# fishmarch/MS-SLAM

Hardware: AMD Instinct MI355X
Metric: Mkeypoints/s extract+describe, KITTI-00-like stereo 1241x376, 2000 feat/frame (higher is better)
Workload: dtype u8

## Files before the change

### ms-slam_amd/csrc/orb_kernels.hip

```cpp
#include <hip/hip_runtime.h>

#include <algorithm>
#include <string>
#include <stdint.h>
#include <stdlib.h>

#include "lds_limit.h"
#include "orb_device.h"
#include "gauss7_stream_device.h"
#include "sincosf_restated.h"

namespace msorb {

__global__ __launch_bounds__(256) void pyr_resize_kernel(LevelView src, LevelView dst, uint8_t* __restrict__ dst_base,
                                                         const ResizeTap* __restrict__ tx,
                                                         const ResizeTap* __restrict__ ty, int single_stage) {
    const int img = blockIdx.z;
    const int dy = blockIdx.y * 4 + (threadIdx.x >> 6);
    const int dx0 = (blockIdx.x * 64 + (threadIdx.x & 63)) * 4;
    if (dy >= dst.h || dx0 >= dst.w) return;
    const ResizeTap vy = ty[dy];
    const uint8_t* s0 = src.base + (size_t)img * src.img_stride + (size_t)vy.i0 * src.pitch;
    const uint8_t* s1 = src.base + (size_t)img * src.img_stride + (size_t)vy.i1 * src.pitch;
    const int b0 = vy.c0, b1 = vy.c1;
// ... 185 lines not shown
    static constexpr int kTileRows = 58;
    static constexpr int kTilePitch = 52;
    static constexpr int kScorePitch = 52;
    static constexpr int kScoreRows = 54;
    static constexpr int kMaxDet = 51;
    static constexpr int kWorkCap = 1536;
    static constexpr int kThreads = 128;
    static constexpr int kWordsPerRow = 2;
    static constexpr int kMaxR = 5;
    static constexpr int kMinWaves = 8;
};

__device__ __forceinline__ int min3i(int a, int b, int c) { return min(a, min(b, c)); }
__device__ __forceinline__ int max3i(int a, int b, int c) { return max(a, max(b, c)); }

#define MSORB_PK2(NAME, OPC)                                                                                                   \
    __device__ __forceinline__ uint32_t NAME(uint32_t a, uint32_t b) {                                                         \
        uint32_t r; asm(OPC " %0, %1, %2" : "=v"(r) : "v"(a), "v"(b)); return r; }                                             \
    __device__ __forceinline__ uint32_t NAME##_sw(uint32_t a, uint32_t b) {                            \
        uint32_t r; asm(OPC " %0, %1, %2 op_sel:[0,1] op_sel_hi:[1,0]" : "=v"(r) : "v"(a), "v"(b)); return r; }
MSORB_PK2(pk_min16, "v_pk_min_i16")
MSORB_PK2(pk_max16, "v_pk_max_i16")
#undef MSORB_PK2
__device__ __forceinline__ uint32_t pk_mad16(uint32_t a, uint32_t b, uint32_t c) {
    uint32_t r; asm("v_pk_mad_i16 %0, %1, %2, %3" : "=v"(r) : "v"(a), "v"(b), "v"(c)); return r;
}

template <class GEO>
__device__ __forceinline__ int fast_arc_contrast_pk(const uint8_t* p, int sgn) {
    constexpr int P = GEO::kTilePitch;
    const uint32_t sv = ((uint32_t)(sgn * (int)p[0]) & 0xffffu) * 0x10001u, ns = ((uint32_t)(-sgn) & 0xffffu) * 0x10001u;
    uint32_t D[8];
    D[0] = pk_mad16(((uint32_t)p[-3 * P] << 16) | p[3 * P], ns, sv);
    D[1] = pk_mad16(((uint32_t)p[-3 * P - 1] << 16) | p[3 * P + 1], ns, sv);
    D[2] = pk_mad16(((uint32_t)p[-2 * P - 2] << 16) | p[2 * P + 2], ns, sv);
    D[3] = pk_mad16(((uint32_t)p[-1 * P - 3] << 16) | p[1 * P + 3], ns, sv);
    D[4] = pk_mad16(((uint32_t)p[-3] << 16) | p[3], ns, sv);
    D[5] = pk_mad16(((uint32_t)p[1 * P - 3] << 16) | p[-1 * P + 3], ns, sv);
    D[6] = pk_mad16(((uint32_t)p[2 * P - 2] << 16) | p[-2 * P + 2], ns, sv);
    D[7] = pk_mad16(((uint32_t)p[3 * P - 1] << 16) | p[-3 * P + 1], ns, sv);
    const uint32_t m2_1 = pk_min16(D[1], D[2]), m2_3 = pk_min16(D[3], D[4]), m2_5 = pk_min16(D[5], D[6]),
                   m2_7 = pk_min16_sw(D[7], D[0]);
    const uint32_t m4_1 = pk_min16(m2_1, m2_3), m4_3 = pk_min16(m2_3, m2_5), m4_5 = pk_min16(m2_5, m2_7),
                   m4_7 = pk_min16_sw(m2_7, m2_1);
    const uint32_t c8_0 = pk_min16(m4_1, m4_5), c8_2 = pk_min16(m4_3, m4_7), c8_4 = pk_min16_sw(m4_5, m4_1),
                   c8_6 = pk_min16_sw(m4_7, m4_3);
    const uint32_t e0 = pk_max16_sw(D[0], D[1]), e2 = pk_max16_sw(D[2], D[3]), e4 = pk_max16_sw(D[4], D[5]),
                   e6 = pk_max16_sw(D[6], D[7]);
    const uint32_t a = pk_max16(pk_max16(pk_min16(c8_0, e0), pk_min16(c8_2, e2)), pk_max16(pk_min16(c8_4, e4), pk_min16(c8_6, e6)));
    return (int)(short)(pk_max16_sw(a, a) & 0xffffu);
}

__device__ __forceinline__ int wave_incl_scan(int v, int) {
    v += __builtin_amdgcn_update_dpp(0, v, 0x111 , 0xf, 0xf, false);
    v += __builtin_amdgcn_update_dpp(0, v, 0x112 , 0xf, 0xf, false);
    v += __builtin_amdgcn_update_dpp(0, v, 0x114 , 0xf, 0xf, false);
    v += __builtin_amdgcn_update_dpp(0, v, 0x118 , 0xf, 0xf, false);
    v += __builtin_amdgcn_update_dpp(0, v, 0x142 , 0xa, 0xf, false);
    v += __builtin_amdgcn_update_dpp(0, v, 0x143 , 0xc, 0xf, false);
    return v;
}

typedef short short2v __attribute__((ext_vector_type(2)));
__device__ __forceinline__ short2v as_s2(uint32_t v) { return __builtin_bit_cast(short2v, v); }
__device__ __forceinline__ uint32_t as_u32(short2v v) { return __builtin_bit_cast(uint32_t, v); }


template <int WAVES>
__device__ __forceinline__ int block_excl_scan(int cnt, int lane, int wave, int* wave_tot , int* total) {
    const int incl = wave_incl_scan(cnt, lane);
    if (lane == 63) wave_tot[wave] = incl;
    __syncthreads();
    int before = 0, tot = 0;
#pragma unroll
    for (int w = 0; w < WAVES; w++) {
        const int c = wave_tot[w];
        if (w < wave) before += c;
        tot += c;
    }
    *total = tot;
    return before + incl - cnt;
}

template <bool ALIGNED, class GEO>
__device__ __forceinline__ void fast_cells_body(const PyramidView& pyr, const CellDesc* __restrict__ cells, const FastThreadRec* __restrict__ ttab,
                                                         int ini_th, int min_th, int slots_per_image,
                                                         Cand16* __restrict__ slots, int* __restrict__ cell_count,
                                                         int n_cells, uint32_t gx_magic, const unsigned lin, const unsigned grid_x, const unsigned total) {
    constexpr int T = GEO::kThreads, P = GEO::kTilePitch, SP = GEO::kScorePitch;
    constexpr int kScoreBytes = (GEO::kScoreRows * SP + 15) & ~15;
    constexpr int kBitWords = GEO::kWordsPerRow * GEO::kMaxDet;
    static_assert(kBitWords <= T, "one bitmap word per thread");
    constexpr FastShape kShape = T == kFastSmall.threads ? kFastSmall : kFastLarge;
    static_assert(kShape.threads == T && kShape.tile_pitch == P && kShape.col_lanes == (P <= 64 ? 16 : 32), "orb_host.h FastShape");
    __shared__ __attribute__((aligned(16))) uint8_t tile_mem[kTileFront + GEO::kTileRows * P + 8];
    __shared__ __attribute__((aligned(16))) uint8_t score[kScoreBytes];
    __shared__ uint16_t work[GEO::kWorkCap];
    __shared__ int wave_tot[2][T / 64];
    __shared__ uint32_t kbits[kBitWords];
    __shared__ int kprefix[kBitWords];
    __shared__ uint16_t lut[32];
    __shared__ uint16_t tbase[T];
    uint8_t* const tile = tile_mem + kTileFront;

    const unsigned chunk = (total + 7) >> 3;
    unsigned wg = (lin & 7u) * chunk + (lin >> 3);
    if (total & 7u) wg = lin;
    const int img = gx_magic ? (int)__umulhi(wg, gx_magic) : (int)(wg / grid_x);
    const int cell_id = (int)(wg - (unsigned)img * grid_x);
    const CellDesc cd = cells[cell_id];
    const LevelView lv = pyr.lv[cd.level];
    const int rw = cd.rw, rh = cd.rh;
    const int dh = rh - 6;
    const int tid = threadIdx.x, lane = tid & 63, wave = tid >> 6;
    const int ga = cd.x0 & ~3;
    const int x_lo = cd.x0 + 3, x_hi = cd.x0 + rw - 3;
    const int gx0 = x_lo & ~3;
    const int G = cd.G;
    const int c_lo = gx0 - ga;
    const uint32_t magic = cd.g_magic;

    const uint8_t* src = lv.base + (size_t)img * lv.img_stride + (size_t)cd.y0 * lv.pitch;
    FastThreadRec tr{};
    if (ALIGNED) tr = ttab[cd.tt_off + (uint32_t)tid];
    if (ALIGNED) {
        constexpr int kColLanes = P <= 64 ? 16 : 32;
        constexpr int kRowsPerPass = T / kColLanes;
        constexpr int kPasses = (GEO::kTileRows - 1 + kRowsPerPass - 1) / kRowsPerPass;
        const int c = tid & (kColLanes - 1), r0 = tid / kColLanes;
        if (c < cd.ndw) {
            const uint32_t col = (uint32_t)(ga + 4 * c);
            const uint32_t pitch = (uint32_t)lv.pitch;
            const uint32_t off0 = __umul24((uint32_t)r0, pitch) + col, off_last = (uint32_t)(rh - 1) * pitch + col;
            uint32_t v[kPasses];
#pragma unroll
            for (int p = 0; p < kPasses; p++)
                v[p] = *reinterpret_cast<const uint32_t*>(src + min(off0 + (uint32_t)(p * kRowsPerPass) * pitch, off_last));
            uint8_t* l0 = &tile[tr.lds_store];
#pragma unroll
            for (int p = 0; p < kPasses; p++)
                if ((p + 1) * kRowsPerPass <= GEO::kTileRows || r0 + p * kRowsPerPass < GEO::kTileRows)
                    *reinterpret_cast<uint32_t*>(l0 + p * kRowsPerPass * P) = v[p];
        }
    } else {
        const int off = cd.x0 - ga;
        const uint32_t bmagic = cd.rw_magic;
        for (int i = tid; i < rh * rw; i += T) {
            const int y = (int)(__umul24((uint32_t)i, bmagic) >> 20), x = i - (int)__umul24((uint32_t)y, (uint32_t)rw);
            tile[(int)__umul24((uint32_t)y, P) + off + x] = src[(size_t)(__umul24((uint32_t)y, (uint32_t)lv.pitch) + (uint32_t)(cd.x0 + x))];
        }
    }
    auto clear_planes = [&]() {
#pragma unroll
        for (int k = 0; k < (kScoreBytes / 16 + T - 1) / T; k++)
            if ((k + 1) * T <= kScoreBytes / 16 || tid + k * T < kScoreBytes / 16)
                reinterpret_cast<uint4*>(score)[tid + k * T] = uint4{0, 0, 0, 0};
        if (tid < kBitWords) kbits[tid] = 0;
    };
    clear_planes();
    if (tid < 32) lut[tid] = (uint16_t)((((tid >> 1) & 3) << 7) + (tid >> 3) + ((tid & 1) << 15));

    const bool by_wave = (T == 128 ? cd.by_wave[0] : cd.by_wave[1]) != 0;
    const int sw = __builtin_amdgcn_readfirstlane(wave) * 8;
    const int R = !by_wave ? (T == 128 ? cd.R128 : cd.R256) : (int)(((T == 128 ? cd.rw128 : cd.rw256) >> sw) & 255u);
    int nrows;
    uint32_t Hm;
    uint32_t colp_off;
    uint32_t baseA;
    if (ALIGNED) {
        nrows = (int)(tr.rows_tbase & 0xffffu);
        Hm = tr.hm;
        colp_off = tr.colp;
        baseA = tr.rows_tbase >> 16;
    } else {
        int g_own, y_b;
        if (!by_wave) {
            const int strip = (int)(__umul24((uint32_t)tid, magic) >> 20);
            g_own = tid - strip * G;
            y_b = strip * R;
        } else {
            const int sl = (int)(__umul24((uint32_t)lane, magic) >> 20);
            g_own = lane - sl * G;
            const int y_w = (int)(((T == 128 ? cd.yw128 : cd.yw256) >> sw) & 255u);
            y_b = sl < (int)cd.spw ? y_w + sl * R : dh;
        }
        nrows = min(max(dh - y_b, 0), R);
        const int c_own = c_lo + 4 * g_own;
        const int xg = ga + c_own;
        const int vlo = min(max(x_lo - xg, 0), 4), vhi = min(max(x_hi - xg, 0), 4);
        Hm = (0x80808080u << (8 * vlo)) & (uint32_t)(0x0080808080ull >> (8 * (4 - vhi)));
        if (vlo >= 4) Hm = 0;
        colp_off = __umul24((uint32_t)y_b, P) + (uint32_t)c_own;
        baseA = (uint32_t)(((y_b + 3) << 7) | c_own);
    }
    tbase[tid] = (uint16_t)baseA;
    auto quick_test = [&](int th, uint32_t& wA, uint32_t& wB) {
        wA = 0; wB = 0;
        const uint8_t* colp = &tile[colp_off];
        uint32_t cw[GEO::kMaxR + 6], lw[GEO::kMaxR], rw_[GEO::kMaxR];
#pragma unroll
        for (int r = 0; r < GEO::kMaxR + 6; r++)
            if (r < 9 || r - 6 < R) cw[r] = *reinterpret_cast<const uint32_t*>(colp + r * P);
#pragma unroll
        for (int k = 0; k < GEO::kMaxR; k++)
            if (k < 3 || k < R) {
                lw[k] = *reinterpret_cast<const uint32_t*>(colp + (k + 3) * P - 4);
                rw_[k] = *reinterpret_cast<const uint32_t*>(colp + (k + 3) * P + 4);
            }
        const ushort2v t2 = __builtin_bit_cast(ushort2v, (uint32_t)th * 0x00010001u);
#pragma unroll
        for (int k = 0; k < GEO::kMaxR; k++) {
            if (k >= 3 && k >= R) break;
            const uint32_t V = cw[k + 3], U = cw[k], D = cw[k + 6];
            const uint32_t R3 = __builtin_amdgcn_alignbyte(rw_[k], V, 3);
            const uint32_t L3 = __builtin_amdgcn_alignbyte(V, lw[k], 1);
            const uint32_t Ve = V & 0x00ff00ffu, Vo = (V >> 8) & 0x00ff00ffu;
            const uint32_t Ae = __builtin_bit_cast(uint32_t, __builtin_elementwise_sub_sat(__builtin_bit_cast(ushort2v, Ve), t2));
            const uint32_t Ao = __builtin_bit_cast(uint32_t, __builtin_elementwise_sub_sat(__builtin_bit_cast(ushort2v, Vo), t2));
            const uint32_t Qd = ~(Ae | (Ao << 8));
            const uint32_t Be = __builtin_bit_cast(uint32_t, __builtin_elementwise_sub_sat(__builtin_bit_cast(ushort2v, Ve ^ 0x00ff00ffu), t2));
            const uint32_t Bo = __builtin_bit_cast(uint32_t, __builtin_elementwise_sub_sat(__builtin_bit_cast(ushort2v, Vo ^ 0x00ff00ffu), t2));
            const uint32_t Qb = Be | (Bo << 8);
            const uint32_t one = 0x01010101u;
            const uint32_t X = (__builtin_amdgcn_lerp(U, Qd, one) & __builtin_amdgcn_lerp(D, Qd, one)) |
                               (__builtin_amdgcn_lerp(L3, Qd, one) & __builtin_amdgcn_lerp(R3, Qd, one));
            const uint32_t Y = (__builtin_amdgcn_lerp(U, Qb, 0u) | __builtin_amdgcn_lerp(D, Qb, 0u)) &
                               (__builtin_amdgcn_lerp(L3, Qb, 0u) | __builtin_amdgcn_lerp(R3, Qb, 0u));
            const uint32_t hm = k < nrows ? Hm : 0u;
            const uint32_t z = (Y & hm) | ((~X & hm) >> 1);
            if (k < 4) wA |= z >> (6 - 2 * k);
            else wB |= z >> (6 - 2 * (k - 4));
        }
    };
    __syncthreads();

    const int sc_off = 4 - c_lo;
    Cand16* const out = slots + (size_t)img * slots_per_image + cd.slot_off;
    int n_emitted = 0;
    for (int pass = 0; pass < 2; pass++) {
        const int th = pass ? min_th : ini_th;
        uint32_t wA, wB;
        quick_test(th, wA, wB);
        const int cnt = __popc(wA) + __popc(wB);
        int n_work = 0;
        const int my_base = block_excl_scan<T / 64>(cnt, lane, wave, wave_tot[0], &n_work);

        const uint32_t baseB = baseA + (4u << 7);
        int w_begin = 0, n_corner = 0;
        if (n_work <= GEO::kWorkCap) {
            uint16_t* wp = &work[my_base];
            const uint32_t idA = (uint32_t)tid << 5, idB = idA | (1u << (5 + (T == 128 ? 7 : 8)));
            for (uint32_t w = wA; w; w &= w - 1) *wp++ = (uint16_t)(idA | (uint32_t)__builtin_ctz(w));
            for (uint32_t w = wB; w; w &= w - 1) *wp++ = (uint16_t)(idB | (uint32_t)__builtin_ctz(w));
            __syncthreads();
            w_begin = wave * ((((n_work + T / 64 - 1) / (T / 64)) + 63) & ~63);
            const int w_end = min(w_begin + ((((n_work + T / 64 - 1) / (T / 64)) + 63) & ~63), n_work);
            n_corner = 0;
            for (int i0 = w_begin; i0 < w_end; i0 += 64) {
                const int i = i0 + lane;
                bool corner = false;
                int ce = 0;
                if (i < w_end) {
                    const int id = work[i];
                    const int e = tbase[(id >> 5) & (T - 1)] + lut[id & 31] + ((id >> (5 + (T == 128 ? 7 : 8))) << 9);
                    const int ty = (e >> 7) & 127, tx = e & 127;
                    const int A = fast_arc_contrast_pk<GEO>(&tile[(int)__umul24((uint32_t)ty, P) + tx], (e & 0x8000) ? -1 : 1);
                    if (A > th) {
                        score[(int)__umul24((uint32_t)(ty - 2), SP) + tx + sc_off] = (uint8_t)(A - 1);
                        ce = e & 0x3FFF;
                        corner = true;
                    }
                }
                const unsigned long long bm = __ballot(corner);
                if (corner)
                    work[w_begin + n_corner + (int)__builtin_amdgcn_mbcnt_hi((uint32_t)(bm >> 32), __builtin_amdgcn_mbcnt_lo((uint32_t)bm, 0u))] = (uint16_t)ce;
                n_corner += __popcll(bm);
            }
        } else {
#pragma unroll 1
            for (int half = 0; half < 2; half++)
#pragma unroll 1
                for (uint32_t w = half ? wB : wA; w; w &= w - 1) {
                    const int e = lut[__builtin_ctz(w)] + (half ? baseB : baseA);
                    const int ty = (e >> 7) & 127, tx = e & 127;
                    const int A = fast_arc_contrast_pk<GEO>(&tile[(int)__umul24((uint32_t)ty, P) + tx], (e & 0x8000) ? -1 : 1);
                    if (A > th) score[(int)__umul24((uint32_t)(ty - 2), SP) + tx + sc_off] = (uint8_t)(A - 1);
                }
        }
        __syncthreads();

        if (n_work <= GEO::kWorkCap) {
            constexpr int wpr = GEO::kWordsPerRow;
            const int nwords = dh * wpr;
            uint32_t mine_keep = 0;
            {
                int slot = 0;
                for (int m0 = 0; m0 < n_corner; m0 += 64, slot++) {
                    if (m0 + lane >= n_corner) continue;
                    const int e = work[w_begin + m0 + lane];
                    const int ty = e >> 7, tx = e & 127;
                    const uint8_t* q = &score[(int)__umul24((uint32_t)(ty - 2), SP) + tx + sc_off];
                    const int sv = q[0];
                    int m = max3i(q[-SP - 1], q[-SP], q[-SP + 1]);
                    m = max3i(m, q[-1], q[1]);
                    m = max(m, max3i(q[SP - 1], q[SP], q[SP + 1]));
                    if (sv > m) {
                        const int bx = tx - c_lo, by = ty - 3;
                        const int b = by * (32 * wpr) + bx;
                        atomicOr(&kbits[b >> 5], 1u << (b & 31));
                        mine_keep |= 1u << slot;
                    }
                }
            }
            __syncthreads();
            const uint32_t myword = tid < nwords ? kbits[tid] : 0u;
            int n_out = 0;
            const int wprefix = block_excl_scan<T / 64>(__popc(myword), lane, wave, wave_tot[1], &n_out);
            if (tid < nwords) kprefix[tid] = wprefix;
            __syncthreads();
            {
                int slot = 0;
                for (int m0 = 0; m0 < n_corner; m0 += 64, slot++) {
                    if (!(mine_keep & (1u << slot))) continue;
                    const int e = work[w_begin + m0 + lane];
                    const int ty = e >> 7, tx = e & 127;
                    const int b = (ty - 3) * (32 * wpr) + (tx - c_lo);
                    const int rank = kprefix[b >> 5] + __popc(kbits[b >> 5] & ((1u << (b & 31)) - 1u));
                    Cand16 c;
                    c.x = (uint16_t)(ga + tx - kMinBorder);
                    c.y = (uint16_t)(cd.y0 + ty - kMinBorder);
                    c.score = score[(int)__umul24((uint32_t)(ty - 2), SP) + tx + sc_off];
                    c.pad = 0;
                    out[rank] = c;
                }
            }
            n_emitted = n_out;
        } else {
            const int n_task = dh * G;
            uint32_t tid_here = (uint32_t)tid;
            asm volatile("" : "+v"(tid_here));
            const int t_begin = (int)(__umul24(tid_here, (uint32_t)n_task) / T),
                      t_end = (int)(__umul24(tid_here + 1u, (uint32_t)n_task) / T);
            uint64_t keep = 0;
            {
                int y = (int)(__umul24((uint32_t)t_begin, magic) >> 20);
                int g = t_begin - y * G;
                for (int task = t_begin, k = 0; task < t_end; task++, k++) {
                    const uint8_t* sp = &score[(y + 1) * SP + 4 + 4 * g];
                    const uint32_t S = *reinterpret_cast<const uint32_t*>(sp);
                    if (S) {
#pragma unroll
                        for (int j = 0; j < 4; j++) {
                            const int sv = (S >> (8 * j)) & 255;
                            if (sv) {
                                const uint8_t* q = sp + j;
                                int m = max3i(q[-SP - 1], q[-SP], q[-SP + 1]);
                                m = max3i(m, q[-1], q[1]);
                                m = max(m, max3i(q[SP - 1], q[SP], q[SP + 1]));
                                if (sv > m) keep |= 1ull << (4 * k + j);
                            }
                        }
                    }
                    if (++g == G) { g = 0; y++; }
                }
            }
            int n_out = 0;
            int pos = block_excl_scan<T / 64>(__popcll(keep), lane, wave, wave_tot[1], &n_out);
            if (keep) {
                int y = (int)(__umul24((uint32_t)t_begin, magic) >> 20);
                int g = t_begin - y * G;
                uint64_t m = keep;
                for (int task = t_begin; task < t_end; task++, m >>= 4) {
                    uint32_t m4 = (uint32_t)m & 15u;
                    while (m4) {
                        const int j = __ffs(m4) - 1;
                        m4 &= m4 - 1;
                        Cand16 c;
                        c.x = (uint16_t)(gx0 + 4 * g + j - kMinBorder);
                        c.y = (uint16_t)(cd.y0 + 3 + y - kMinBorder);
                        c.score = score[(y + 1) * SP + 4 + 4 * g + j];
                        c.pad = 0;
                        out[pos++] = c;
                    }
                    if (++g == G) { g = 0; y++; }
                }
            }
            n_emitted = n_out;
        }
        if (n_emitted > 0 || pass == 1 || ini_th == min_th) break;
        __syncthreads();
        clear_planes();
        __syncthreads();
    }
    if (tid == 0) cell_count[(size_t)img * n_cells + cell_id] = n_emitted;
}

template <bool ALIGNED, class GEO>
__global__ __launch_bounds__(GEO::kThreads, GEO::kMinWaves) void fast_cells_kernel(PyramidView pyr, const CellDesc* __restrict__ cells,
                                                         const FastThreadRec* __restrict__ ttab,
                                                         int ini_th, int min_th, int slots_per_image,
                                                         Cand16* __restrict__ slots, int* __restrict__ cell_count,
                                                         int n_cells, uint32_t gx_magic) {
    fast_cells_body<ALIGNED, GEO>(pyr, cells, ttab, ini_th, min_th, slots_per_image, slots, cell_count, n_cells, gx_magic,
                                  blockIdx.y * gridDim.x + blockIdx.x, gridDim.x, gridDim.x * gridDim.y);
}

__global__ __launch_bounds__(256) void cand_scan_cells_kernel(const int* __restrict__ cell_count, int n_cells,
                                                              const int* __restrict__ level_cell_begin, int nlevels,
                                                              int* __restrict__ cell_off, int* __restrict__ level_count,
                                                              int* __restrict__ img_total, int* __restrict__ img_base,
                                                              int fixed_stride) {
    __shared__ int wave_tot[4];
    __shared__ int lvl[kMaxLevels];
    const int img = blockIdx.x, tid = threadIdx.x, lane = tid & 63, wave = tid >> 6;
    if (fixed_stride > 0 && tid == 0) {
        img_base[img] = img * fixed_stride;
        if (img == (int)gridDim.x - 1) img_base[gridDim.x] = (int)gridDim.x * fixed_stride;
    }
    const int* cnt = cell_count + (size_t)img * n_cells;
    int* off = cell_off + (size_t)img * n_cells;
    const int per = (n_cells + 255) / 256;
    const int b = tid * per, e = min(b + per, n_cells);
    constexpr int kCache = 4;
    int c[kCache];
#pragma unroll
    for (int k = 0; k < kCache; k++) c[k] = b + k < e ? cnt[b + k] : 0;
    int s = 0;
#pragma unroll
    for (int k = 0; k < kCache; k++) s += c[k];
    for (int i = b + kCache; i < e; i++) s += cnt[i];
    if (tid < kMaxLevels) lvl[tid] = 0;
    int total = 0;
    int acc = block_excl_scan<4>(s, lane, wave, wave_tot, &total);
    if (tid == 0) img_total[img] = total;
    int cur_l = 0, cur_t = 0;
    auto visit = [&](int i, int v) {
        off[i] = acc;
        acc += v;
        while (i >= level_cell_begin[cur_l + 1]) {
            if (cur_t) atomicAdd(&lvl[cur_l], cur_t);
            cur_t = 0;
            cur_l++;
        }
        cur_t += v;
    };
#pragma unroll
    for (int k = 0; k < kCache; k++)
        if (b + k < e) visit(b + k, c[k]);
    for (int i = b + kCache; i < e; i++) visit(i, cnt[i]);
    if (cur_t) atomicAdd(&lvl[cur_l], cur_t);
    __syncthreads();
    if (tid < nlevels) level_count[(size_t)img * nlevels + tid] = lvl[tid];
}

__global__ __launch_bounds__(256) void cand_scan_images_kernel(const int* __restrict__ img_total, int n_images,
                                                               int* __restrict__ img_base ) {
    __shared__ int wave_tot[4];
    const int tid = threadIdx.x, lane = tid & 63, wave = tid >> 6;
    const int per = (n_images + 255) / 256;
    const int b = tid * per, e = min(b + per, n_images);
    const int first = b < e ? img_total[b] : 0;
    int s = first;
    for (int i = b + 1; i < e; i++) s += img_total[i];
    int total = 0;
    int acc = block_excl_scan<4>(s, lane, wave, wave_tot, &total);
    if (tid == 0) img_base[n_images] = total;
    if (b < e) { img_base[b] = acc; acc += first; }
    for (int i = b + 1; i < e; i++) { img_base[i] = acc; acc += img_total[i]; }
}

constexpr int kGatherThreads = 256;
constexpr int kGatherCells = kGatherThreads / 16;
__global__ __launch_bounds__(kGatherThreads) void cand_gather_kernel(const CellDesc* __restrict__ cells, int n_cells,
                                                          int slots_per_image, const Cand16* __restrict__ slots,
                                                          const int* __restrict__ cell_count,
                                                          const int* __restrict__ cell_off,
                                                          const int* __restrict__ img_base, Cand16* __restrict__ compact) {
    const int c0 = blockIdx.x * kGatherCells + 2 * (int)(threadIdx.x >> 5), img = blockIdx.y, l = threadIdx.x & 31;
    if (c0 >= n_cells) return;
    const int c1 = min(c0 + 1, n_cells - 1);
    const int* cnt = cell_count + (size_t)img * n_cells;
    const int* off = cell_off + (size_t)img * n_cells;
    const int n0 = cnt[c0], n1 = c0 + 1 < n_cells ? cnt[c1] : 0;
    const int o0 = off[c0], o1 = off[c1], s0 = cells[c0].slot_off, s1 = cells[c1].slot_off, base = img_base[img];
    const Cand16* sp = slots + (size_t)img * slots_per_image;
    Cand16* d = compact + base;
    Cand16 v0{}, v1{};
// ... 88 lines not shown
    if (ALIGNED) {
        const uint32_t* ap = reinterpret_cast<const uint32_t*>(rp + x0);
        w1 = ap[0]; w2 = ap[1];
        w0 = x0 ? ap[-1] : 0u;
    } else {
        const uint32_t ph = (uint32_t)(reinterpret_cast<uintptr_t>(rp) & 3);
        const uint32_t* ap = reinterpret_cast<const uint32_t*>(rp - ph + x0);
        const uint32_t d1 = ap[0], d2 = ap[1], d3 = ap[2];
        const uint32_t d0 = x0 ? ap[-1] : 0u;
        w0 = __builtin_amdgcn_alignbyte(d1, d0, ph);
        w1 = __builtin_amdgcn_alignbyte(d2, d1, ph);
        w2 = __builtin_amdgcn_alignbyte(d3, d2, ph);
    }
    if (x0 == 0) w0 = __builtin_amdgcn_perm(0u, w1, 0x01020300u);
#pragma unroll
    for (int j = 0; j < 4; j++) {
        const uint32_t a = j == 3 ? w1 : __builtin_amdgcn_alignbyte(w1, w0, j + 1);
        const uint32_t b = j == 3 ? w2 : __builtin_amdgcn_alignbyte(w2, w1, j + 1);
        hsum[j] = __builtin_amdgcn_udot4(b, kGaussHi, __builtin_amdgcn_udot4(a, kGaussLo, 0u, false), false);
    }
}

template <bool ALIGNED>
__global__ __launch_bounds__(256) void gauss7_kernel(PyramidView src, PyramidView dst, BlurPlan plan, GaussTaps T) {
    const uint32_t K[7] = {T.k[0], T.k[1], T.k[2], T.k[3], T.k[4], T.k[5], T.k[6]};
    const uint32_t kGaussLo = K[0] | (K[1] << 8) | (K[2] << 16) | (K[3] << 24), kGaussHi = K[4] | (K[5] << 8) | (K[6] << 16);
    int level = 0;
    while (level + 1 < plan.nlevels && (int)blockIdx.x >= plan.block_begin[level + 1]) level++;
    const int rem = blockIdx.x - plan.block_begin[level];
    const int bx = rem % plan.bx_count[level], by = rem / plan.bx_count[level];
    const LevelView sv = src.lv[level], dv = dst.lv[level];
    const int img = blockIdx.y;
    const int x0 = (bx * 64 + (threadIdx.x & 63)) * 4;
    const int y0 = (by * 4 + (threadIdx.x >> 6)) * kGaussRows;
    if (x0 + 16 > sv.w || y0 >= sv.h) return;
    const uint8_t* sb = sv.base + (size_t)img * sv.img_stride;
    uint8_t* db = const_cast<uint8_t*>(dv.base) + (size_t)img * dv.img_stride;
    uint32_t acc[7][4];
    uint32_t hs[4];
#pragma unroll
    for (int r = 0; r < 6; r++) {
        gauss_row_sums<ALIGNED>(sb, sv.pitch, sv.h, y0 - 3 + r, x0, hs, kGaussLo, kGaussHi);
#pragma unroll
        for (int t = 0; t <= r; t++)
#pragma unroll
            for (int j = 0; j < 4; j++) acc[r - t][j] = (t == 0 ? 0u : acc[r - t][j]) + K[t] * hs[j];
    }
    for (int it = 0; it < kGaussRows / 7; it++) {
#pragma unroll
        for (int u = 0; u < 7; u++) {
            const int r = 6 + 7 * it + u;
            gauss_row_sums<ALIGNED>(sb, sv.pitch, sv.h, y0 - 3 + r, x0, hs, kGaussLo, kGaussHi);
#pragma unroll
            for (int t = 0; t < 7; t++) {
                const int a = (6 + u - t) % 7;
#pragma unroll
                for (int j = 0; j < 4; j++) acc[a][j] = (t == 0 ? 0u : acc[a][j]) + K[t] * hs[j];
            }
            const int o = r - 6, a = u % 7;
            if (y0 + o < sv.h) {
                uint32_t packed = 0;
#pragma unroll
                for (int j = 0; j < 4; j++) packed |= min((acc[a][j] + 32768u) >> 16, 255u) << (8 * j);
                *reinterpret_cast<uint32_t*>(db + blur_tile_off((uint32_t)x0, (uint32_t)(y0 + o), (uint32_t)dv.pitch)) = packed;
            }
        }
    }
}

template <int ROWS>
__global__ __launch_bounds__(256) void gauss7_stream_kernel(PyramidView src, PyramidView dst, BlurPlan plan, int per_xcd,
                                                            int total_blocks) {
    const int tile = (int)(blockIdx.x & 7u) * per_xcd + (int)(blockIdx.x >> 3);
    if (tile >= total_blocks) return;
    gauss7_stream_body<ROWS>(src, dst, plan, tile, (int)(threadIdx.x >> 6));
}

template <bool ALIGNED, class GEO>
__global__ __launch_bounds__(GEO::kThreads) void frame_fast_blur_kernel(PyramidView pyr, const CellDesc* __restrict__ cells, const FastThreadRec* __restrict__ ttab, int ini_th, int min_th,
                                                                        int slots_per_image, Cand16* __restrict__ slots, int* __restrict__ cell_count,
                                                                        int n_cells, uint32_t gx_magic, unsigned n_fast, PyramidView blur, BlurPlan plan,
                                                                        int blur_blocks) {
    if (blockIdx.x < n_fast) {
        fast_cells_body<ALIGNED, GEO>(pyr, cells, ttab, ini_th, min_th, slots_per_image, slots, cell_count, n_cells, gx_magic, blockIdx.x, (unsigned)n_cells, n_fast);
        return;
    }
    constexpr int kWavesPerWg = GEO::kThreads / 64, kWgPerTile = 4 / kWavesPerWg;
    const unsigned b = blockIdx.x - n_fast;
    const int tile = (int)(b / kWgPerTile);
    if (tile >= blur_blocks) return;
    gauss7_stream_body<kGaussRows>(pyr, blur, plan, tile, (int)(b % kWgPerTile) * kWavesPerWg + (int)(threadIdx.x >> 6));
}

constexpr int kEdgeRows = 58;
__global__ __launch_bounds__(64) void gauss7_edge_kernel(PyramidView src, PyramidView dst, GaussTaps T) {
    __shared__ uint16_t hs[64][16];
    const int level = blockIdx.y, img = blockIdx.z;
    const LevelView sv = src.lv[level], dv = dst.lv[level];
    const int first = sv.w >= 16 ? ((sv.w - 16) / 4 + 1) * 4 : 0;
    const int ncol = sv.w - first;
    const int y0 = blockIdx.x * kEdgeRows;
    if (y0 >= sv.h) return;
    const int r = threadIdx.x;
    const uint8_t* sb = sv.base + (size_t)img * sv.img_stride;
    uint8_t* db = const_cast<uint8_t*>(dv.base) + (size_t)img * dv.img_stride;
    const int K[7] = {(int)T.k[0], (int)T.k[1], (int)T.k[2], (int)T.k[3], (int)T.k[4], (int)T.k[5], (int)T.k[6]};
    {
        int yy = refl101(y0 - 3 + r, sv.h);
        yy = min(max(yy, 0), sv.h - 1);
        const uint8_t* rp = sb + (size_t)yy * sv.pitch;
        uint32_t px[22];
#pragma unroll
        for (int o = 0; o < 22; o++) px[o] = rp[min(max(refl101(first - 3 + o, sv.w), 0), sv.w - 1)];
#pragma unroll
        for (int j = 0; j < 16; j++) {
            uint32_t a = 0;
#pragma unroll
            for (int k = 0; k < 7; k++) a += K[k] * px[j + k];
            hs[r][j] = (uint16_t)a;
        }
    }
    __syncthreads();
    if (r < kEdgeRows && y0 + r < sv.h) {
        for (int j = 0; j < ncol; j++) {
            uint32_t acc = 0;
#pragma unroll
            for (int k = 0; k < 7; k++) acc += (uint32_t)K[k] * hs[r + k][j];
            db[blur_tile_off((uint32_t)(first + j), (uint32_t)(y0 + r), (uint32_t)dv.pitch)] = (uint8_t)min((acc + 32768u) >> 16, 255u);
        }
    }
}

struct PatchTables {
    int8_t pattern[256 * 4];
    int8_t umax[16];
};
__constant__ PatchTables c_tab;

void upload_patch_tables(const int8_t* pattern, const int* umax, hipStream_t stream) {
    PatchTables t;
    for (int i = 0; i < 1024; i++) t.pattern[i] = pattern[i];
    for (int v = 0; v <= kHalfPatch; v++) t.umax[v] = (int8_t)umax[v];
    (void)hipMemcpyToSymbolAsync(HIP_SYMBOL(c_tab), &t, sizeof(t), 0, hipMemcpyHostToDevice, stream);
    (void)hipStreamSynchronize(stream);
}

hipError_t download_patch_tables(int8_t* pattern, int8_t* umax, hipStream_t stream) {
    PatchTables t;
    hipError_t e = hipMemcpyFromSymbolAsync(&t, HIP_SYMBOL(c_tab), sizeof(t), 0, hipMemcpyDeviceToHost, stream);
    if (e == hipSuccess) e = hipStreamSynchronize(stream);
    if (e != hipSuccess) return e;
    memcpy(pattern, t.pattern, sizeof(t.pattern));
    memcpy(umax, t.umax, sizeof(t.umax));
    return hipSuccess;
}

__device__ __forceinline__ float fast_atan2_deg(float y, float x, int fma) {
    const float scale = (float)(180 / 3.1415926535897932384626433832795);
    const float p1 = 0.9997878412794807f * scale, p3 = -0.3258083974640975f * scale;
    const float p5 = 0.1555786518463281f * scale, p7 = -0.04432655554792128f * scale;
    const float eps = (float)2.2204460492503131e-16;
    const float ax = fabsf(x), ay = fabsf(y);
    float a, c, c2;
    auto poly = [&](float cc, float cc2) {
        if (fma) return __fmul_rn(__fmaf_rn(__fmaf_rn(__fmaf_rn(p7, cc2, p5), cc2, p3), cc2, p1), cc);
        return __fmul_rn(__fadd_rn(__fmul_rn(__fadd_rn(__fmul_rn(__fadd_rn(__fmul_rn(p7, cc2), p5), cc2), p3), cc2), p1), cc);
    };
// ... 502 lines not shown
            *reinterpret_cast<uint32_t*>(dbuf + r * dp + 4 * c) = packed;
            if (dy >= oy0 && dy < oy1 && dx0 >= ox0 && dx0 < ox1) *reinterpret_cast<uint32_t*>(dplane + (size_t)dy * dpitch + dx0) = packed;
        }
        __syncthreads();
    }
}

bool build_tower_plan(TowerPlan& plan, int nlevels, const int* w, const int* h, const int* pitch, const std::vector<std::vector<ResizeTap>>& taps_x,
                      const std::vector<std::vector<ResizeTap>>& taps_y, size_t lds_limit) {
    plan = TowerPlan{};
    if (nlevels < 2) return false;
    const int ntx = kTowerTiles, nty = w[0] >= 2 * h[0] ? kTowerTiles / 2 : kTowerTiles;
    for (int l = 0; l < nlevels; l++)
        if (pitch[l] < ((w[l] + 3) & ~3)) return false;
    size_t lds[2] = {0, 0};
    for (int tyi = 0; tyi < kTowerTiles; tyi++)
        for (int l = nlevels - 1; l >= 0; l--) {
            int a = l ? tower_own_y(tyi, nty, h[l]) : 32767, b = l ? tower_own_y(tyi + 1, nty, h[l]) : -1;
            if (l + 1 < nlevels && plan.y[l + 1].need1[tyi] > plan.y[l + 1].need0[tyi]) {
                const auto& t = taps_y[l + 1];
                a = std::min<int>(a, t[plan.y[l + 1].need0[tyi]].i0);
                b = std::max<int>(b, t[std::min<int>(plan.y[l + 1].need1[tyi], h[l + 1]) - 1].i1 + 1);
            }
            if (b <= a) { a = 0; b = 0; }
            plan.y[l].need0[tyi] = (int16_t)a; plan.y[l].need1[tyi] = (int16_t)b;
        }
    for (int txi = 0; txi < kTowerTiles; txi++)
        for (int l = nlevels - 1; l >= 0; l--) {
            int a = l ? tower_own_x(txi, ntx, w[l]) : 32767, b = l ? tower_own_x(txi + 1, ntx, w[l]) : -1;
            if (l + 1 < nlevels && plan.x[l + 1].need1[txi] > plan.x[l + 1].need0[txi]) {
                const auto& t = taps_x[l + 1];
                a = std::min<int>(a, t[std::min<int>(plan.x[l + 1].need0[txi], w[l + 1] - 1)].i0);
                b = std::max<int>(b, (t[std::min<int>(plan.x[l + 1].need1[txi], w[l + 1]) - 1].i1 + 1));
            }
            if (b <= a) { a = 0; b = 0; }
            a &= ~3; b = (b + 3) & ~3;
            plan.x[l].need0[txi] = (int16_t)a; plan.x[l].need1[txi] = (int16_t)b;
        }
    for (int l = 0; l < nlevels; l++)
        for (int tyi = 0; tyi < nty; tyi++)
            for (int txi = 0; txi < ntx; txi++) {
                const size_t bytes = (size_t)(plan.x[l].need1[txi] - plan.x[l].need0[txi] + 8) * (plan.y[l].need1[tyi] - plan.y[l].need0[tyi]) + 16;
                lds[l & 1] = std::max(lds[l & 1], (bytes + 15) & ~size_t(15));
            }
    size_t n_taps = 0;
    for (int tyi = 0; tyi < nty; tyi++)
        for (int txi = 0; txi < ntx; txi++) {
            size_t t = 0;
            for (int l = 1; l < nlevels; l++) t += (size_t)(plan.x[l].need1[txi] - plan.x[l].need0[txi]) + ((plan.y[l].need1[tyi] - plan.y[l].need0[tyi] + 1) & ~1);
            n_taps = std::max(n_taps, t);
        }
    if (n_taps > 2048 || lds[0] + lds[1] + (n_taps + 8) * sizeof(ResizeTap) > lds_limit) return false;
    plan.ntx = ntx; plan.nty = nty;
    plan.lds_even = (int)lds[0]; plan.lds_odd = (int)lds[1]; plan.lds_taps = (int)((n_taps + 8) * sizeof(ResizeTap));
    return true;
}
bool launch_pyramid_tower(const PyramidView& pyr, const TowerPlan& plan, const ResizeTap* taps, const size_t* tap_x_off, const size_t* tap_y_off,
                          int n_images, hipStream_t s) {
    static const bool off = getenv("MSORB_PYR_TOWER") && atoi(getenv("MSORB_PYR_TOWER")) == 0;
    const LevelView& v0 = pyr.lv[0];
    if (off || plan.ntx <= 0 || (reinterpret_cast<uintptr_t>(v0.base) & 3) || (v0.pitch & 3) || (v0.img_stride & 3) || v0.pitch < ((v0.w + 3) & ~3) ||
        (reinterpret_cast<uintptr_t>(taps) & 31))
        return false;
    const size_t lds = (size_t)plan.lds_even + plan.lds_odd + plan.lds_taps;
    if ((long long)lds > dynamic_lds_room(reinterpret_cast<const void*>(pyr_tower_kernel))) return false;
    TowerTaps t{};
    for (int l = 1; l < pyr.nlevels; l++) { t.x[l] = taps + tap_x_off[l]; t.y[l] = taps + tap_y_off[l]; }
    hipLaunchKernelGGL(pyr_tower_kernel, dim3(plan.ntx, plan.nty, n_images), dim3(kTowerThreads), lds, s, pyr, plan, t);
    return true;
}
void launch_pyramid(const PyramidView& pyr, const ResizeTap* taps, const size_t* tap_x_off, const size_t* tap_y_off, int n_images,
                    hipStream_t s, const Semantics& sem) {
    for (int l = 1; l < pyr.nlevels; l++)
        launch_pyr_resize(pyr.lv[l - 1], pyr.lv[l], const_cast<uint8_t*>(pyr.lv[l].base), taps + tap_x_off[l], taps + tap_y_off[l], n_images, s,
                          sem.resize_single_stage);
}
void launch_fast_cells(const PyramidView& pyr, const CellDesc* cells, const FastThreadRec* ttab, int n_cells, int ini_th, int min_th,
                       int slots_per_image, Cand16* slots, int* cell_count, int n_images, bool small_cells, hipStream_t s) {
    bool aligned = true;
    for (int l = 0; l < pyr.nlevels; l++) {
        const LevelView& v = pyr.lv[l];
        aligned = aligned && (reinterpret_cast<uintptr_t>(v.base) & 3) == 0 && (v.pitch & 3) == 0 && (v.img_stride & 3) == 0;
    }
    const dim3 grid(n_cells, n_images);
    const uint32_t gx_magic = exact_div_magic((unsigned)n_cells, (unsigned long long)n_cells * (unsigned)n_images);
#define MSORB_FAST_LAUNCH(AL, GEO)                                                                                        \
    hipLaunchKernelGGL((fast_cells_kernel<AL, GEO>), grid, dim3(GEO::kThreads), 0, s, pyr, cells, ttab, ini_th, min_th, slots_per_image, slots, \
                       cell_count, n_cells, gx_magic)
    if (small_cells) { if (aligned) MSORB_FAST_LAUNCH(true, GeoSmall); else MSORB_FAST_LAUNCH(false, GeoSmall); }
    else { if (aligned) MSORB_FAST_LAUNCH(true, GeoLarge); else MSORB_FAST_LAUNCH(false, GeoLarge); }
#undef MSORB_FAST_LAUNCH
}
void launch_cand_compact(const CellDesc* cells, int n_cells, const int* level_cell_begin, int nlevels,
                         int slots_per_image, const Cand16* slots, const int* cell_count, int* cell_off,
                         int* level_count, int* img_total, int* img_base, Cand16* compact, int n_images,
                         hipStream_t s, bool packed, bool frame_form) {
    if (!packed && frame_form && n_images <= 4 && n_cells <= kFrameCompactCells) {
        hipLaunchKernelGGL(cand_compact_frame_kernel, dim3((n_cells + kGatherCells - 1) / kGatherCells, n_images), dim3(kGatherThreads), 0, s, cells, n_cells,
                           level_cell_begin, nlevels, slots_per_image, slots, cell_count, cell_off, level_count, img_total, img_base, compact);
        return;
    }
    hipLaunchKernelGGL(cand_scan_cells_kernel, dim3(n_images), dim3(256), 0, s, cell_count, n_cells, level_cell_begin,
                       nlevels, cell_off, level_count, img_total, img_base, packed ? 0 : slots_per_image);
    if (packed) hipLaunchKernelGGL(cand_scan_images_kernel, dim3(1), dim3(256), 0, s, img_total, n_images, img_base);
    hipLaunchKernelGGL(cand_gather_kernel, dim3((n_cells + kGatherCells - 1) / kGatherCells, n_images), dim3(kGatherThreads), 0, s, cells, n_cells, slots_per_image,
                       slots, cell_count, cell_off, img_base, compact);
}
static bool levels_aligned(const PyramidView& v) {
    bool aligned = true;
    for (int l = 0; l < v.nlevels; l++) {
        const LevelView& lv = v.lv[l];
        aligned = aligned && (reinterpret_cast<uintptr_t>(lv.base) & 3) == 0 && (lv.pitch & 3) == 0 && (lv.img_stride & 3) == 0;
    }
    return aligned;
}
static BlurPlan make_blur_plan(const PyramidView& src, int n_images, bool stream, int* total_out, int* max_h_out) {
    BlurPlan plan{};
    plan.nlevels = src.nlevels;
    const int rows = kGaussRows;
    int total = 0, max_h = 0;
    for (int l = 0; l < src.nlevels; l++) {
        const LevelView& v = src.lv[l];
        plan.block_begin[l] = total;
        const int main_groups = stream ? (v.w + 3) / 4 : (v.w >= 16 ? (v.w - 16) / 4 + 1 : 0);
        plan.bx_count[l] = stream ? max(1, (main_groups - 1 + kGaussLanesOut - 1) / kGaussLanesOut) : (v.w + 255) / 256;
        const int strips = (v.h + rows - 1) / rows;
        total += plan.bx_count[l] * ((strips + 3) / 4);
        max_h = max(max_h, v.h);
    }
    plan.block_begin[src.nlevels] = total;
    for (int l = 0; l < src.nlevels; l++)
        plan.bx_magic[l] = exact_div_magic((unsigned)plan.bx_count[l], (unsigned long long)(plan.block_begin[l + 1] - plan.block_begin[l]));
    for (int l = src.nlevels; l < kMaxLevels; l++) plan.bx_magic[l] = 0;
    plan.image_magic = exact_div_magic((unsigned)total, (unsigned long long)total * (unsigned)n_images + 8);
    *total_out = total;
    *max_h_out = max_h;
    return plan;
}
int launch_gauss7(const PyramidView& src, const PyramidView& dst, int n_images, hipStream_t s, const Semantics& sem) {
    const bool aligned = levels_aligned(src);
    const bool stream = aligned && sem.default_taps();
    GaussTaps T;
    for (int i = 0; i < 7; i++) T.k[i] = (uint32_t)sem.gauss_taps[i];
    int total = 0, max_h = 0;
    const BlurPlan plan = make_blur_plan(src, n_images, stream, &total, &max_h);
    if (stream) {
        const int all = total * n_images, per_xcd = (all + 7) / 8;
        hipLaunchKernelGGL(gauss7_stream_kernel<kGaussRows>, dim3(per_xcd * 8), dim3(256), 0, s, src, dst, plan, per_xcd, all);
    }
    else if (aligned) hipLaunchKernelGGL(gauss7_kernel<true>, dim3(total, n_images), dim3(256), 0, s, src, dst, plan, T);
    else hipLaunchKernelGGL(gauss7_kernel<false>, dim3(total, n_images), dim3(256), 0, s, src, dst, plan, T);
    if (!stream)
        hipLaunchKernelGGL(gauss7_edge_kernel, dim3((max_h + kEdgeRows - 1) / kEdgeRows, src.nlevels, n_images), dim3(64), 0, s, src, dst, T);
    return 0;
}
bool make_frame_blur_job(const PyramidView& src, const PyramidView& dst, int n_images, const Semantics& sem, FrameBlurJob* job) {
    if (!levels_aligned(src) || !sem.default_taps()) return false;
    int total = 0, max_h = 0;
    job->src = src; job->dst = dst;
    job->plan = make_blur_plan(src, n_images, true, &total, &max_h);
    job->blocks = total * n_images;
    return true;
}
bool launch_frame_fast_blur(const PyramidView& pyr, const PyramidView& blur, const CellDesc* cells, const FastThreadRec* ttab, int n_cells, int ini_th, int min_th,
                            int slots_per_image, Cand16* slots, int* cell_count, int n_images, bool small_cells, hipStream_t s,
                            const Semantics& sem) {
    if (!levels_aligned(pyr) || !sem.default_taps()) return false;
    int total = 0, max_h = 0;
// ... 29 lines not shown
```

Baseline: 495.9.

## Process runs of consecutive FAST cells per workgroup with prefetched descriptors

The FAST cell kernel now has each workgroup loop over up to four consecutive cells instead of one, so the grid shrinks by that factor. Per-thread table records and derived row/column state are reloaded only when the cell class changes, and the next cell descriptor is prefetched into scalar registers while the current cell is processed. This amortises launch, descriptor-load and setup cost across cells, at the price of fewer workgroups for the GPU to spread across CUs and serial work inside each one. The tile store is also rewritten to clamp spare rows instead of using a predicate.

```diff
diff --git a/ms-slam_amd/csrc/orb_kernels.hip b/ms-slam_amd/csrc/orb_kernels.hip
--- a/ms-slam_amd/csrc/orb_kernels.hip
+++ b/ms-slam_amd/csrc/orb_kernels.hip
@@ -291,7 +291,23 @@
     return before + incl - cnt;
 }
 
-template <bool ALIGNED, class GEO>
+struct __attribute__((may_alias)) CellWords { uint32_t w[sizeof(CellDesc) / 4]; };
+static_assert(sizeof(CellDesc) % 4 == 0 && alignof(CellDesc) >= 4, "CellDesc is read as dwords");
+__device__ __forceinline__ CellWords load_cell_words(const CellDesc* __restrict__ cells, int id) {
+    return *reinterpret_cast<const CellWords*>(cells + id);
+}
+__device__ __forceinline__ CellDesc cell_of_words(CellWords cw) {
+#pragma unroll
+    for (unsigned i = 0; i < sizeof(CellDesc) / 4; i++) asm("" : "+s"(cw.w[i]));
+    return __builtin_bit_cast(CellDesc, cw);
+}
+
+#ifndef MSORB_FAST_RUN
+#define MSORB_FAST_RUN 4
+#endif
+constexpr int kFastRun = MSORB_FAST_RUN;
+
+template <bool ALIGNED, class GEO, int C>
 __device__ __forceinline__ void fast_cells_body(const PyramidView& pyr, const CellDesc* __restrict__ cells, const FastThreadRec* __restrict__ ttab,
                                                          int ini_th, int min_th, int slots_per_image,
                                                          Cand16* __restrict__ slots, int* __restrict__ cell_count,
@@ -316,12 +332,35 @@
     unsigned wg = (lin & 7u) * chunk + (lin >> 3);
     if (total & 7u) wg = lin;
     const int img = gx_magic ? (int)__umulhi(wg, gx_magic) : (int)(wg / grid_x);
-    const int cell_id = (int)(wg - (unsigned)img * grid_x);
-    const CellDesc cd = cells[cell_id];
-    const LevelView lv = pyr.lv[cd.level];
+    const int cell_first = (int)(wg - (unsigned)img * grid_x) * C;
+    const int cell_end = min(cell_first + C, n_cells);
+    {
+        const int t = threadIdx.x;
+        if (t < 32) lut[t] = (uint16_t)((((t >> 1) & 3) << 7) + (t >> 3) + ((t & 1) << 15));
+    }
+
+    FastThreadRec tr{};
+    int nrows = 0;
+    uint32_t Hm = 0;
+    uint32_t colp_off = 0;
+    uint32_t baseA = 0;
+
+    CellDesc cd = cell_of_words(load_cell_words(cells, cell_first));
+    LevelView lv = pyr.lv[cd.level];
+    uint32_t cur_class = cd.tt_off;
+    if (ALIGNED) tr = ttab[cd.tt_off + threadIdx.x];
+    bool fresh = true;
+#pragma unroll 1
+    for (int cell_id = cell_first;;) {
+    int tid = threadIdx.x;
+    if (!ALIGNED) asm volatile("" : "+v"(tid));
+    const int lane = tid & 63, wave = tid >> 6;
+    const int sw = __builtin_amdgcn_readfirstlane(wave) * 8;
+    const bool more = C > 1 && cell_id + 1 < cell_end;
+    CellWords next_words = {};
+    if (ALIGNED && more) next_words = load_cell_words(cells, cell_id + 1);
     const int rw = cd.rw, rh = cd.rh;
     const int dh = rh - 6;
-    const int tid = threadIdx.x, lane = tid & 63, wave = tid >> 6;
     const int ga = cd.x0 & ~3;
     const int x_lo = cd.x0 + 3, x_hi = cd.x0 + rw - 3;
     const int gx0 = x_lo & ~3;
@@ -329,9 +368,14 @@
     const int c_lo = gx0 - ga;
     const uint32_t magic = cd.g_magic;
 
+    if (ALIGNED && cd.tt_off != cur_class) {
+        cur_class = cd.tt_off;
+        fresh = true;
+        tr = ttab[cd.tt_off + (uint32_t)tid];
+    }
+    if (!ALIGNED) fresh = true;
+
     const uint8_t* src = lv.base + (size_t)img * lv.img_stride + (size_t)cd.y0 * lv.pitch;
-    FastThreadRec tr{};
-    if (ALIGNED) tr = ttab[cd.tt_off + (uint32_t)tid];
     if (ALIGNED) {
         constexpr int kColLanes = P <= 64 ? 16 : 32;
         constexpr int kRowsPerPass = T / kColLanes;
@@ -345,11 +389,13 @@
 #pragma unroll
             for (int p = 0; p < kPasses; p++)
                 v[p] = *reinterpret_cast<const uint32_t*>(src + min(off0 + (uint32_t)(p * kRowsPerPass) * pitch, off_last));
+            static_assert(GEO::kTileRows - 1 >= GEO::kMaxDet + 6, "the tile's last row is spare");
             uint8_t* l0 = &tile[tr.lds_store];
 #pragma unroll
-            for (int p = 0; p < kPasses; p++)
-                if ((p + 1) * kRowsPerPass <= GEO::kTileRows || r0 + p * kRowsPerPass < GEO::kTileRows)
-                    *reinterpret_cast<uint32_t*>(l0 + p * kRowsPerPass * P) = v[p];
+            for (int p = 0; p < kPasses; p++) {
+                if ((p + 1) * kRowsPerPass <= GEO::kTileRows) *reinterpret_cast<uint32_t*>(l0 + p * kRowsPerPass * P) = v[p];
+                else *reinterpret_cast<uint32_t*>(l0 + min(p * kRowsPerPass, GEO::kTileRows - 1 - r0) * P) = v[p];
+            }
         }
     } else {
         const int off = cd.x0 - ga;
@@ -359,6 +405,39 @@
             tile[(int)__umul24((uint32_t)y, P) + off + x] = src[(size_t)(__umul24((uint32_t)y, (uint32_t)lv.pitch) + (uint32_t)(cd.x0 + x))];
         }
     }
+    const bool by_wave = (T == 128 ? cd.by_wave[0] : cd.by_wave[1]) != 0;
+    const int R = !by_wave ? (T == 128 ? cd.R128 : cd.R256) : (int)(((T == 128 ? cd.rw128 : cd.rw256) >> sw) & 255u);
+    if (fresh) {
+        fresh = false;
+        if (ALIGNED) {
+            nrows = (int)(tr.rows_tbase & 0xffffu);
+            Hm = tr.hm;
+            colp_off = tr.colp;
+            baseA = tr.rows_tbase >> 16;
+        } else {
+            int g_own, y_b;
+            if (!by_wave) {
+                const int strip = (int)(__umul24((uint32_t)tid, magic) >> 20);
+                g_own = tid - strip * G;
+                y_b = strip * R;
+            } else {
+                const int sl = (int)(__umul24((uint32_t)lane, magic) >> 20);
+                g_own = lane - sl * G;
+                const int y_w = (int)(((T == 128 ? cd.yw128 : cd.yw256) >> sw) & 255u);
+                y_b = sl < (int)cd.spw ? y_w + sl * R : dh;
+            }
+            nrows = min(max(dh - y_b, 0), R);
+            const int c_own = c_lo + 4 * g_own;
+            const int xg = ga + c_own;
+            const int vlo = min(max(x_lo - xg, 0), 4), vhi = min(max(x_hi - xg, 0), 4);
+            Hm = (0x80808080u << (8 * vlo)) & (uint32_t)(0x0080808080ull >> (8 * (4 - vhi)));
+            if (vlo >= 4) Hm = 0;
+            colp_off = __umul24((uint32_t)y_b, P) + (uint32_t)c_own;
+            baseA = (uint32_t)(((y_b + 3) << 7) | c_own);
+        }
+        tbase[tid] = (uint16_t)baseA;
+    }
+    __syncthreads();
     auto clear_planes = [&]() {
 #pragma unroll
         for (int k = 0; k < (kScoreBytes / 16 + T - 1) / T; k++)
@@ -367,42 +446,7 @@
         if (tid < kBitWords) kbits[tid] = 0;
     };
     clear_planes();
-    if (tid < 32) lut[tid] = (uint16_t)((((tid >> 1) & 3) << 7) + (tid >> 3) + ((tid & 1) << 15));
-
-    const bool by_wave = (T == 128 ? cd.by_wave[0] : cd.by_wave[1]) != 0;
-    const int sw = __builtin_amdgcn_readfirstlane(wave) * 8;
-    const int R = !by_wave ? (T == 128 ? cd.R128 : cd.R256) : (int)(((T == 128 ? cd.rw128 : cd.rw256) >> sw) & 255u);
-    int nrows;
-    uint32_t Hm;
-    uint32_t colp_off;
-    uint32_t baseA;
-    if (ALIGNED) {
-        nrows = (int)(tr.rows_tbase & 0xffffu);
-        Hm = tr.hm;
-        colp_off = tr.colp;
-        baseA = tr.rows_tbase >> 16;
-    } else {
-        int g_own, y_b;
-        if (!by_wave) {
-            const int strip = (int)(__umul24((uint32_t)tid, magic) >> 20);
-            g_own = tid - strip * G;
-            y_b = strip * R;
-        } else {
-            const int sl = (int)(__umul24((uint32_t)lane, magic) >> 20);
-            g_own = lane - sl * G;
-            const int y_w = (int)(((T == 128 ? cd.yw128 : cd.yw256) >> sw) & 255u);
-            y_b = sl < (int)cd.spw ? y_w + sl * R : dh;
-        }
-        nrows = min(max(dh - y_b, 0), R);
-        const int c_own = c_lo + 4 * g_own;
-        const int xg = ga + c_own;
-        const int vlo = min(max(x_lo - xg, 0), 4), vhi = min(max(x_hi - xg, 0), 4);
-        Hm = (0x80808080u << (8 * vlo)) & (uint32_t)(0x0080808080ull >> (8 * (4 - vhi)));
-        if (vlo >= 4) Hm = 0;
-        colp_off = __umul24((uint32_t)y_b, P) + (uint32_t)c_own;
-        baseA = (uint32_t)(((y_b + 3) << 7) | c_own);
-    }
-    tbase[tid] = (uint16_t)baseA;
+
     auto quick_test = [&](int th, uint32_t& wA, uint32_t& wB) {
         wA = 0; wB = 0;
         const uint8_t* colp = &tile[colp_off];
@@ -441,7 +485,6 @@
             else wB |= z >> (6 - 2 * (k - 4));
         }
     };
-    __syncthreads();
 
     const int sc_off = 4 - c_lo;
     Cand16* const out = slots + (size_t)img * slots_per_image + cd.slot_off;
@@ -602,6 +645,13 @@
         __syncthreads();
     }
     if (tid == 0) cell_count[(size_t)img * n_cells + cell_id] = n_emitted;
+    if (!more) break;
+    cell_id++;
+    const int level = cd.level;
+    if (!ALIGNED) next_words = load_cell_words(cells, cell_id);
+    cd = cell_of_words(next_words);
+    if (cd.level != level) lv = pyr.lv[cd.level];
+    }
 }
 
 template <bool ALIGNED, class GEO>
@@ -610,8 +660,8 @@
                                                          int ini_th, int min_th, int slots_per_image,
                                                          Cand16* __restrict__ slots, int* __restrict__ cell_count,
                                                          int n_cells, uint32_t gx_magic) {
-    fast_cells_body<ALIGNED, GEO>(pyr, cells, ttab, ini_th, min_th, slots_per_image, slots, cell_count, n_cells, gx_magic,
-                                  blockIdx.y * gridDim.x + blockIdx.x, gridDim.x, gridDim.x * gridDim.y);
+    fast_cells_body<ALIGNED, GEO, kFastRun>(pyr, cells, ttab, ini_th, min_th, slots_per_image, slots, cell_count, n_cells, gx_magic,
+                                            blockIdx.y * gridDim.x + blockIdx.x, gridDim.x, gridDim.x * gridDim.y);
 }
 
 __global__ __launch_bounds__(256) void cand_scan_cells_kernel(const int* __restrict__ cell_count, int n_cells,
@@ -866,7 +916,7 @@
                                                                         int n_cells, uint32_t gx_magic, unsigned n_fast, PyramidView blur, BlurPlan plan,
                                                                         int blur_blocks) {
     if (blockIdx.x < n_fast) {
-        fast_cells_body<ALIGNED, GEO>(pyr, cells, ttab, ini_th, min_th, slots_per_image, slots, cell_count, n_cells, gx_magic, blockIdx.x, (unsigned)n_cells, n_fast);
+        fast_cells_body<ALIGNED, GEO, 1>(pyr, cells, ttab, ini_th, min_th, slots_per_image, slots, cell_count, n_cells, gx_magic, blockIdx.x, (unsigned)n_cells, n_fast);
         return;
     }
     constexpr int kWavesPerWg = GEO::kThreads / 64, kWgPerTile = 4 / kWavesPerWg;
@@ -1535,8 +1585,9 @@
         const LevelView& v = pyr.lv[l];
         aligned = aligned && (reinterpret_cast<uintptr_t>(v.base) & 3) == 0 && (v.pitch & 3) == 0 && (v.img_stride & 3) == 0;
     }
-    const dim3 grid(n_cells, n_images);
-    const uint32_t gx_magic = exact_div_magic((unsigned)n_cells, (unsigned long long)n_cells * (unsigned)n_images);
+    const unsigned n_runs = ((unsigned)n_cells + kFastRun - 1) / kFastRun;
+    const dim3 grid(n_runs, n_images);
+    const uint32_t gx_magic = exact_div_magic(n_runs, (unsigned long long)n_runs * (unsigned)n_images);
 #define MSORB_FAST_LAUNCH(AL, GEO)                                                                                        \
     hipLaunchKernelGGL((fast_cells_kernel<AL, GEO>), grid, dim3(GEO::kThreads), 0, s, pyr, cells, ttab, ini_th, min_th, slots_per_image, slots, \
                        cell_count, n_cells, gx_magic)
```

Result: slower. 490.2 (-1.1%).
